# pymlex/recommendation-system-pokec

Measured on AMD Instinct MI355X. Metric: FAS candidates scored/sec over 1.6M users, top-k=10; 1/2/4/8 GPU + %HBM peak, higher is better.
Workload: dtype f64; 1 GPU; cfg2: full 1.6M-user single-query interest FAS all-candidates top-10; workload_key=cfg2_all_candidates_top10_1632803users_q1_shard1of1, topk=10, parallelism=candidate-shard x1, hw_queues=4

## Files before the change

include/pokec_fas.h:

```cpp
#ifndef POKEC_FAS_H
#define POKEC_FAS_H

#include <stdint.h>

#ifdef __cplusplus
extern "C" {
#endif

#define PF_ABI_VERSION 2

#define PF_OK          0
#define PF_EINVAL     -1
#define PF_ENODEV     -2
#define PF_ENOMEM     -3
#define PF_ENOTFOUND  -4
#define PF_EUNSUPP    -5
#define PF_EINTERNAL  -6

#define PF_NUM_FIXED   7
#define PF_MAX_COLS    64
#define PF_F_PUBLIC     0
#define PF_F_GENDER     1
#define PF_F_COMPLETION 2
#define PF_F_AGE        3
// ... 190 lines not shown
                       int32_t topk, uint64_t* d_keys, void* stream);
int pf_merge_keys_async(pf_ctx* ctx, const uint64_t* d_parts, int32_t nparts,
                        int32_t nq, int32_t topk, uint64_t* d_out, void* stream);
void pf_decode_keys(const uint64_t* keys, int32_t n, int32_t* out_uid,
                    float* out_score, int32_t* count);

typedef struct pf_layout_stats {
    int64_t n_slots;
    int64_t stream_bytes;
    int64_t header_bytes;
    int64_t alg_bytes;
    int32_t packed_tokens;
    int32_t n_tiles;
    int64_t post_bytes;
    int32_t scan_kernel;
    int32_t resident_images;
    int64_t shard_cands;
    int64_t shard_entries;
} pf_layout_stats;
int pf_layout(const pf_ctx* ctx, pf_layout_stats* out);

int pf_scan_bytes(pf_ctx* ctx, const int32_t* query_uid, int32_t nq, int64_t* out_bytes);
int pf_scan_prune_stats(pf_ctx* ctx, int64_t* out, int32_t reset);

typedef struct pf_jobs_stats {
    int64_t jobs, candidates, pairs;
    int64_t pair_alg_bytes, pair_record_bytes, pair_image_bytes;
    double  pair_ms;
    int64_t pair_launches;
    int64_t pair_dispatches;
} pf_jobs_stats;
int pf_jobs_stats_reset(pf_ctx* ctx, int32_t enable);
int pf_jobs_stats_read(pf_ctx* ctx, pf_jobs_stats* out);

float pf_last_scan_ms(const pf_ctx* ctx);
int pf_profile_reset(pf_ctx* ctx);
int pf_profile_read(pf_ctx* ctx, double* total_ms, int64_t* launches);
int pf_profile_sample(pf_ctx* ctx, int32_t every);

#ifdef __cplusplus
}
#endif
#endif
```

recommendation-system-pokec_amd/csrc/pf_api.cpp:

```cpp
#include <hip/hip_runtime.h>

#include <algorithm>
#include <atomic>
#include <cmath>
#include <cstdlib>
#include <cstring>
#include <mutex>
#include <string>
#include <thread>
#include <unordered_map>
#include <unordered_set>
#include <vector>

#include "pf_batch.h"
#include "pf_ctx.h"
#include "pf_debug.h"
#include "pf_kernels.h"
#include "pf_store.h"
#include "pokec_fas.h"

using pf::DBuf;
using pf::PinBuf;
using pf::Ranked;
using pf::par_jobs;
// ... 243 lines not shown
        HIPCHK(c, hipStreamSynchronize(c->stream));
        k.hl.lap(pf::kHpGpu);
        const pf_pair_terms_head* rh = c->h_thead.as<pf_pair_terms_head>();
        const double* rt = c->h_terms.as<double>();
        par_jobs(k.g1 - k.g0, [&](size_t i) {
            const size_t g = k.g0 + i;
            for (size_t j = 0; j < slots[g].size(); ++j) {
                head[dest[g][j]] = rh[k.gf[i] + j];
                std::memcpy(terms + (size_t)dest[g][j] * W, rt + (k.gf[i] + j) * W, W * sizeof(double));
            }
        }, 256);
        k.hl.lap(pf::kHpUnpack);
        return PF_OK;
    });
}

uint32_t post_mode(bool claimed) {
    static const long pr = pf::debug_long("k5_prune", 2);
    static const bool prb = pf::debug_long("k5_prune_batch", 1) != 0;
    static const bool prs = pf::debug_long("k5_prune_stats", 0) != 0;
    const uint32_t p = pr <= 0 ? 0u : (pf::kPostPrune | (pr == 1 ? pf::kPostPruneBlockOnly : 0u) | (prs ? pf::kPostPruneStats : 0u));
    static const bool fko = pf::debug_long("k5_filter_blockout", 1) == 0;
    const uint32_t f = fko ? pf::kPostFiltKeepBlocks : 0u;
    return ((claimed || prb) ? p : 0u) | f;
}

constexpr int kBatchBlocksPerWgDefault = 32;
int batch_blocks_per_wg() {
    static const int n = (int)std::max(1L, pf::debug_long("k5_batch_blocks", kBatchBlocksPerWgDefault));
    return n;
}

uint32_t post_image_lds(const pf::QPostHead* h) {
    return pf::post_lds(pf::post_var_lds(h->n_tok, h->n_tok + h->n_club + h->n_friend));
}
uint32_t filt_lds(const pf_ctx* c) { return (c->filt.fields ? pf::kFiltLds : 0u) + (c->win.fields ? pf::kWinLds : 0u); }

struct CountScope {
    pf_ctx* c;
    int n;
    bool on;
    CountScope(pf_ctx* ctx, int nq) : c(ctx), n(nq), on((ctx->win.fields & pf::kWinCount) != 0u && nq > 0) {}
    ~CountScope() { c->cur_totals = nullptr; }
    int begin() {
        if (!on) return PF_OK;
        HIPCHK(c, c->d_totals.ensure((size_t)n * sizeof(uint32_t)));
        HIPCHK(c, hipMemsetAsync(c->d_totals.p, 0, (size_t)n * sizeof(uint32_t), c->stream));
// ... 1262 lines not shown
}

int pf_merge_keys_async(pf_ctx* c, const uint64_t* d_parts, int32_t nparts, int32_t nq, int32_t topk, uint64_t* d_out,
                        void* stream) {
    if (!c || nparts < 1 || nq < 0 || topk <= 0 || topk > pf::kMaxTopK) return PF_EINVAL;
    (void)hipSetDevice(c->device);
    hipStream_t s = (hipStream_t)stream;
    HIPCHK(c, pf::launch_merge(d_parts, nparts, (int64_t)nq * topk, topk, nq, topk, d_out, s));
    return PF_OK;
}

int pf_jobs_stats_reset(pf_ctx* c, int32_t enable) { return c ? pf::jobs_stats_reset(c, enable) : PF_EINVAL; }
int pf_jobs_stats_read(pf_ctx* c, pf_jobs_stats* o) { return (c && o) ? pf::jobs_stats_read(c, o) : PF_EINVAL; }

int pf_scan_prune_stats(pf_ctx* c, int64_t* out, int32_t reset) {
    if (!c || !out) return PF_EINVAL;
    (void)hipSetDevice(c->device);
    unsigned long long v[5];
    HIPCHK(c, pf::k5_prune_stats_read(v, reset != 0));
    for (int i = 0; i < 5; ++i) out[i] = (int64_t)v[i];
    return PF_OK;
}

int pf_scan_bytes(pf_ctx* c, const int32_t* q, int32_t nq, int64_t* out) {
    if (!c || nq < 0 || (nq && (!q || !out))) return PF_EINVAL;
    (void)hipSetDevice(c->device);
    int64_t k1 = 0;
    for (int32_t t = c->tile_begin; t < c->tile_end; ++t) k1 += (int64_t)c->hs.tile_steps[t] * pf::kTileSlots * 16;
    k1 += (int64_t)(c->tile_end - c->tile_begin) * pf::kTileSlots * 48;
    if (!c->use_post()) {
        for (int i = 0; i < nq; ++i) out[i] = c->hc.idx_of(q[i]) < 0 ? 0 : k1;
        return PF_OK;
    }
    std::vector<std::vector<uint8_t>> imgs((size_t)nq);
    std::vector<int8_t> kind((size_t)nq, 0);
    par_jobs((size_t)nq, [&](size_t i) {
        const int32_t x = c->hc.idx_of(q[i]);
        if (x < 0) return;
        std::vector<int32_t> ex;
        auto it = c->hc.adj.find(q[i]);
        if (it != c->hc.adj.end()) ex = it->second;
        ex.push_back(q[i]);
        pf::build_query_post(c->hc, c->hp, x, ex, imgs[i]);
        const pf::QPostHead* h = reinterpret_cast<const pf::QPostHead*>(imgs[i].data() + sizeof(pf::QConst));
        kind[i] = post_image_lds(h) <= kK5LdsCap ? 1 : 2;
    }, 1);
// ... 106 lines not shown
```

recommendation-system-pokec_amd/csrc/pf_kernels.h:

```cpp
#pragma once
#include <hip/hip_runtime.h>

#include "pf_filter.h"
#include "pf_select.h"
#include "pf_types.h"
#include "pf_window.h"

namespace pf {

constexpr int kPairThreads = 512;
struct PairBlock {
    int32_t qimg, begin, count, out;
};

struct PairGen {
    int32_t nf, nch, cap, cand, fl, stride, out, first;
};

struct ScanLaunch {
    const DevStore& st;
    const uint8_t* pool;
    const QImageRef* refs_dev;
    uint32_t lds;
    bool gtab;
    int nq, tile_begin, tile_end, k, blocks;
    uint64_t *parts, *out;
    ScanSync* sync;
    const int32_t* out_rows;
    hipStream_t s;
    const CandFilter& filt;
    const FieldSel& sel;
    const ScanWindow& win;
    uint32_t* totals;
};
hipError_t launch_scan(const ScanLaunch& L);
int scan_blocks_per_cu(bool packed, bool gtab, uint32_t lds);
uint32_t post_var_lds(int n_tok, int n_lists);
uint32_t post_lds(uint32_t var_lds);
constexpr uint32_t kPostPrune = 1u << 16, kPostPruneStats = 1u << 17, kPostPruneBlockOnly = 1u << 18;
constexpr uint32_t kPostFiltKeepBlocks = 1u << 19;
constexpr uint32_t kFiltLds = (uint32_t)sizeof(CandFilter);
static_assert(kFiltLds % 16 == 0, "the window's words follow the filter's");
constexpr uint32_t kWinLds = 32;
static_assert(sizeof(ScanWindow) <= kWinLds, "the window's LDS");
struct PostLaunch {
    const PostStore& ps;
    const uint8_t* pool;
    const uint32_t* img_off;
    uint32_t var_lds;
    int nq, blk_begin, blk_end, k, blocks;
    uint64_t *parts, *out;
    ScanSync* sync;
    const int32_t* out_rows;
    bool claimed;
    uint32_t mode;
    hipEvent_t e0, e1;
    hipStream_t s;
    const uint8_t* qconst;
    const CandFilter& filt;
    const FieldSel& sel;
    const ScanWindow& win;
    uint32_t* totals;
};
hipError_t launch_post(const PostLaunch& L);
int post_blocks_per_cu(uint32_t var_lds, bool claimed, bool filtered, bool selected, bool windowed);
hipError_t launch_filter_count(const PostStore& ps, const DevStore& st, int32_t i0, int32_t i1, const CandFilter& filt,
                               unsigned long long* count, hipStream_t s);
hipError_t k5_prune_stats_read(unsigned long long* out, bool reset);
hipError_t launch_merge(const uint64_t* in, int nparts, int64_t part_stride, int64_t query_stride, int nq, int k,
                        uint64_t* out, hipStream_t s);
struct PairsLaunch {
    const DevStore& st;
    const uint8_t* pool;
    const QImageRef* refs_dev;
    uint32_t max_lds;
    bool gtab;
    const PairBlock* blocks;
    int nblocks;
    const int32_t *order, *slots;
    float* out;
    hipStream_t s;
    const FieldSel& sel;
};
hipError_t launch_pairs(const PairsLaunch& L);
constexpr int kTermsThreads = 256;
constexpr int kTermsPairs = 32;
struct TermsLaunch {
    const DevStore& st;
    const uint8_t* pool;
    const QImageRef* refs_dev;
    uint32_t lds;
// ... 13 lines not shown
```

recommendation-system-pokec_amd/csrc/pf_kernels.hip:

```cpp
#include <hip/hip_ext.h>
#include <hip/hip_runtime.h>

#include <cstdint>
#include <algorithm>
#include <unordered_map>
#include <vector>
#include <cstdio>
#include <cstdlib>

#include "pf_device.h"
#include "pf_filter.h"
#include "pf_kernels.h"
#include "pf_plan.h"
#include "pf_prune.h"
#include "pf_select.h"

namespace pf {

static_assert(sizeof(QConst) % 16 == 0, "QConst must keep the LDS carve 16-B aligned");
static_assert(sizeof(QVal) == 16, "QVal is one 16-B load");

#ifdef PF_K5_TIMERS
__device__ unsigned long long g_k5t[16];
__device__ unsigned long long g_k1t[12];
#endif

constexpr int kPruneStats = 5;
static_assert(kPruneBins <= (int)(sizeof(ScanSync::hist) / sizeof(unsigned int)), "the histogram holds every bin");
__device__ unsigned long long g_k5_prune[kPruneStats];

#ifdef PF_K5_BLOCKLOG
constexpr unsigned kBlogCap = 16384;
__device__ unsigned long long g_blog_t[2 * kBlogCap];
__device__ unsigned int g_blog_meta[kBlogCap];
__device__ unsigned int g_blog_n;
#endif

__device__ __forceinline__ void wave_sync() {
    __builtin_amdgcn_fence(__ATOMIC_RELEASE, "wavefront");
    __builtin_amdgcn_wave_barrier();
    __builtin_amdgcn_fence(__ATOMIC_ACQUIRE, "wavefront");
}

struct Walk {
    uint32_t cnt;
    uint32_t nh;
    uint32_t pend;
};

template <bool PACKED>
struct HitT;
template <>
// ... 790 lines not shown
    double wq, idf;
};

constexpr uint32_t kLdsMask = 0;
constexpr uint32_t kLdsSlot = kLdsMask + 8 * kBlockCands;
constexpr uint32_t kLdsHit = kLdsSlot + 8 * kRoundCap;
constexpr uint32_t kLdsHbase = kLdsHit + 2 * kRoundCap;
constexpr uint32_t kLdsCnt = kLdsSlot;
constexpr uint32_t kLdsExb = kLdsCnt + 4 * kBlockCands;
static_assert(4 * kBlockCands + 4 * (kBlockCands / 32) <= 8 * kRoundCap, "set counters alias the slots");
constexpr uint32_t kLdsItem = kLdsHbase + 2 * kBlockCands;
constexpr uint32_t kLdsMisc = (kLdsItem + 2 * kRoundCap + 15) & ~15u;
constexpr uint32_t kLdsCols = kLdsMisc + 64;
constexpr uint32_t kLdsFtab = kLdsCols + 16 * kPostMaxCols;
constexpr uint32_t kLdsSeg = kLdsFtab + 8 * (kNumFixed + kPostMaxCols + 1);
constexpr uint32_t kLdsCidx = kLdsSeg + 4 * kRoundToks;
constexpr uint32_t kMapWords = kRoundCap / 64;
constexpr uint32_t kLdsMapB = (kLdsCidx + 7) & ~7u;
constexpr uint32_t kLdsMapN = kLdsMapB + 2 * 8 * kMapWords;
constexpr uint32_t kLdsMapC = kLdsMapN + 2 * 8 * kRoundToks;
constexpr uint32_t kLdsLmk = (kLdsMapC + 2 * kMapWords + 7) & ~7u;
constexpr uint32_t kLdsCpre = kLdsLmk + 8 * kPostMaxCols;
constexpr uint32_t kLdsNeed = kLdsCpre + 8 * (kPostMaxCols + 1);
constexpr uint32_t kPostFixedLds = (kLdsNeed + 8 * (kNumFixed + kPostMaxCols + 1) + 15) & ~15u;
static_assert(kBlockCands == 2 * kPostThreads, "two candidates per thread");
static_assert(kRoundCap < 65536 && kBlockCands <= kRoundCap, "u16 slots; a one-token round fits");
static_assert(kPostWaves * kMaxTopK * 8 + 16 + 4 * kMaxTopK <= 8 * kRoundCap, "post_tail scratch in the slots");

constexpr uint32_t kHitFirst = 1u << 14;
constexpr uint32_t kHitCand = 1u << 15;
constexpr uint32_t kSegSplit = 1u << 24;
constexpr uint8_t kColDead = 0xFFu;

#ifdef PF_K5_CHECK
__device__ __forceinline__ uint32_t k5_chk(uint32_t i, uint32_t n, int what) {
    if (i >= n) {
        printf("K5 CHECK %d: index %u >= %u (block %d thread %d)\n", what, i, n, (int)blockIdx.x, (int)threadIdx.x);
        return 0u;
    }
    return i;
}
#define K5CHK(i, n, w) k5_chk((i), (n), (w))
#else
#define K5CHK(i, n, w) (i)
#endif


// ... 176 lines not shown
    uint16_t* hit = reinterpret_cast<uint16_t*>(base + kLdsHit);
    uint16_t* hbase = reinterpret_cast<uint16_t*>(base + kLdsHbase);
    uint16_t* item = reinterpret_cast<uint16_t*>(base + kLdsItem);
    uint32_t* cnt = reinterpret_cast<uint32_t*>(base + kLdsCnt);
    uint32_t* exb = reinterpret_cast<uint32_t*>(base + kLdsExb);
    uint32_t* misc = reinterpret_cast<uint32_t*>(base + kLdsMisc);
    QCol* scol = reinterpret_cast<QCol*>(base + kLdsCols);
    double* ftab = reinterpret_cast<double*>(base + kLdsFtab);
    uint32_t* seg = reinterpret_cast<uint32_t*>(base + kLdsSeg);
    const int nsets = H.n_club + H.n_friend;
    const int nl = H.n_tok + nsets;
    PTok* pt = reinterpret_cast<PTok*>(base + kPostFixedLds);
    uint2* rng = reinterpret_cast<uint2*>(pt + H.n_tok);
    uint2* rtab = rng + nl;
    uint32_t* gpre = reinterpret_cast<uint32_t*>(rtab + H.n_tok + 1);
    uint32_t* spre = gpre + H.n_tok + 1;
    uint8_t* colof = reinterpret_cast<uint8_t*>(spre + nsets + 1);
    uint64_t* mapb = reinterpret_cast<uint64_t*>(base + kLdsMapB);
    uint2* mapn = reinterpret_cast<uint2*>(base + kLdsMapN);
    uint8_t* mapc = reinterpret_cast<uint8_t*>(base + kLdsMapC);
    uint64_t* lmk = reinterpret_cast<uint64_t*>(base + kLdsLmk);
    uint64_t* cpre = reinterpret_cast<uint64_t*>(base + kLdsCpre);
    double* need = reinterpret_cast<double*>(base + kLdsNeed);
    const bool prune = (mode & kPostPrune) != 0u;
    const bool prune_rnd = prune && !(mode & kPostPruneBlockOnly);
    const bool pstats = (mode & kPostPruneStats) != 0u;
    const bool drop = FILT || prune;
    CandFilter* fl = reinterpret_cast<CandFilter*>(
        smem + (((uint32_t)(reinterpret_cast<char*>(colof) + H.n_tok - smem) + 15u) & ~15u));
    if constexpr (FILT) {
        if (tid == 0) *fl = F;
    }
    const ScanWindow* wl = reinterpret_cast<const ScanWindow*>(reinterpret_cast<char*>(fl) + (FILT ? kFiltLds : 0u));
    if constexpr (WIN) {
        if (tid == 0) *const_cast<ScanWindow*>(wl) = W;
    }
    if (tid < 16) misc[tid] = 0u;
    stage(smem, qcp, sizeof(QConst));
    if constexpr (!SEL) {
        for (int j = tid; j < H.n_act; j += kPostThreads) {
            const QCol c = cols[j];
            scol[j] = c;
            for (int x = c.j0; x < c.j1; ++x) colof[x] = (uint8_t)j;
        }
        if (tid == 0) {
            uint64_t m = 0;
            for (int j = 0; j < H.n_act; ++j) { cpre[j] = m; m |= 1ull << cols[j].t; }
            cpre[H.n_act] = m;
        }
// ... 41 lines not shown
    const uint32_t B = (uint32_t)ps.bsize;
    const uint32_t cend = min((uint32_t)blk_end * B, (uint32_t)ps.n);
    const bool short_excl = H.n_excl <= kPostThreads;
    const uint32_t ex0 = short_excl && H.n_excl > 0 ? excl[min(tid, H.n_excl - 1)] : ~0u;
    const int pb = (nbx & 7) == 0 ? (bx & 7) * (nbx >> 3) + (bx >> 3) : bx;
    const int xng = min(8, nbx), xg = bx % xng;
    const int x_lo = blk_begin + (int)((int64_t)(blk_end - blk_begin) * xg / xng);
    const int x_hi = blk_begin + (int)((int64_t)(blk_end - blk_begin) * (xg + 1) / xng);
    const int x_nwg = (nbx - xg + xng - 1) / xng;
    unsigned int* xctr = &sync[qy].xcd_next[xg * 16];
    const int blk_last = XD ? x_hi : blk_end;
    for (int blk = XD ? x_lo + bx / xng : blk_begin + pb; blk < blk_last;) {
        unsigned int xclaim = 0;
        auto next_block = [&](bool now) __attribute__((always_inline)) {
            if constexpr (XD) {
                if (tid == 0) misc[0] = (uint32_t)(x_lo + x_nwg) + (now ? atomicAdd(xctr, 1u) : xclaim);
                __syncthreads();
                blk = (int)misc[0];
            } else {
                __syncthreads();
                blk += nbx;
            }
        };
        const uint32_t c0 = (uint32_t)blk * B;
        const uint32_t c1 = min(c0 + B, cend) - 1;
#ifdef PF_K5_BLOCKLOG
        const unsigned long long blog_t0 = __builtin_amdgcn_s_memrealtime();
#endif
        uint4 ha[kCandsPerThread], hb[kCandsPerThread];
#pragma unroll
        for (int kk = 0; kk < kCandsPerThread; ++kk) {
            const uint32_t c = min(c0 + kk * kPostThreads + tid, c1);
            ha[kk] = ps.hdr[2 * (size_t)c];
            hb[kk] = ps.hdr[2 * (size_t)c + 1];
        }
        uint32_t thb = 0u;
        if (prune) thb = __hip_atomic_load(&sync[qy].theta, __ATOMIC_RELAXED, __HIP_MEMORY_SCOPE_AGENT);
        if constexpr (WIN) {
            if (prune) thb = max(thb, wl->theta0);
        }
#pragma unroll 1
        for (int j = tid; j < nl; j += kPostThreads)
            rng[j] = list_range(ps, j < H.n_tok ? toks[j].l : sets[j - H.n_tok], c0, c1);
#pragma unroll
        for (int kk = 0; kk < kCandsPerThread; ++kk) {
            const uint32_t c = c0 + kk * kPostThreads + tid;
// ... 24 lines not shown
                    misc[12] += thb == 0u ? 1u : 0u;
                }
                next_block(true);
                continue;
            }
#pragma unroll
            for (int kk = 0; kk < kCandsPerThread; ++kk) {
                const uint64_t bal = __ballot((fskip >> kk) & 1u);
                const uint32_t w = (uint32_t)(bal >> (lane & 32));
                if ((lane & 31) == 0 && w != 0u) atomicOr(&exb[(kk * kPostThreads + tid) >> 5], w);
            }
        } else {
            __syncthreads();
        }
        K5T(1);
        if (prune && tid >= kPostThreads - 64) {
            thb = (uint32_t)__builtin_amdgcn_readfirstlane((int)thb);
            const uint32_t rec = misc[5];
            if (rec != 0u) {
                thb = prune_derive(sync + qy, thb | (uint32_t)k, rec);
                wave_sync();
                if (lane == 0) misc[5] = 0u;
            }
            const int u = tid - (kPostThreads - 64);
            if (u == 0) misc[4] = thb;
            if (u >= 0 && u <= kNumFixed + kPostMaxCols) need[u] = prune_need(thb, u, kNumFixed + q.n_cols);
        }
        if (tid < 64) {
            ColPlan cpl = col_tokens(scol, H.n_act, lane);
            wave_prefix<SEL>(gpre, rng, H.n_tok, lane, pt);
            wave_sync();
            col_ends(cpl, gpre, H.n_act, lane);
            {
                int ci0 = 0, j0 = 0, nr = 0;
                while (ci0 < H.n_act) {
                    if constexpr (SEL) j0 = max(j0, __builtin_amdgcn_readlane(cpl.j0, ci0));
                    const Round Rr = plan_round(cpl, gpre, H.n_act, lane, ci0, j0);
                    if (lane == 0)
                        rtab[nr] = make_uint2((uint32_t)Rr.ja | (uint32_t)Rr.jb << 16, (uint32_t)Rr.ca | (uint32_t)Rr.ce << 16);
                    if (nr == 0) build_map(mapb, mapc, mapn, gpre, rng, Rr.ja, Rr.jb, lane);
                    ++nr;
                }
                if (lane == 0) misc[3] = (uint32_t)nr;
            }
        }
        if (short_excl) {
            const uint32_t p = ex0 - c0;
            if (tid < H.n_excl && p < B) atomicOr(&exb[p >> 5], 1u << (p & 31));
        } else {
            uint32_t lo = 0, hi = (uint32_t)H.n_excl;
            while (lo < hi) {
                const uint32_t mid = (lo + hi) >> 1;
                if (excl[mid] < c0) lo = mid + 1; else hi = mid;
            }
            hi = (uint32_t)H.n_excl;
// ... 50 lines not shown
        }
        if (drop) {
#pragma unroll
            for (int kk = 0; kk < kCandsPerThread; ++kk) {
                const bool sk = (skip >> kk) & 1u;
                const bool d = prune && !sk && prune_dead(sum[kk], (double)__popcll(pend[kk]), need[(used >> (8 * kk)) & 0xFFu]);
                if (sk || d) {
                    skip |= 1u << kk;
                    pend[kk] = 0ull;
                }
                if (pstats) {
                    const int p = kk * kPostThreads + tid;
                    const uint64_t bs = __ballot((uint32_t)p < B && c0 + p <= c1), bd = __ballot(d);
                    if (lane == 0) {
                        atomicAdd(&misc[8], (uint32_t)__popcll(bs));
                        atomicAdd(&misc[9], (uint32_t)__popcll(bd));
                    }
                }
            }
            if (pstats && tid == 0) {
                misc[11] += 1u;
                misc[12] += misc[4] == 0u ? 1u : 0u;
            }
        }
        K5T(3);
        double cdot[kCandsPerThread], cnrm[kCandsPerThread];
        uint32_t chit = 0;
#pragma unroll
        for (int kk = 0; kk < kCandsPerThread; ++kk) { cdot[kk] = 0.0; cnrm[kk] = 0.0; }
        int nrounds = (int)misc[3];
        if (XD && nrounds == 0 && tid == 0) xclaim = atomicAdd(xctr, 1u);
        for (int rnd = 0; rnd < nrounds; ++rnd) {
            if (XD && rnd == nrounds - 1 && tid == 0) xclaim = atomicAdd(xctr, 1u);
            const uint2 rr = rtab[rnd];
            Round R;
            R.ja = (int)(rr.x & 0xFFFFu);
            R.jb = (int)(rr.x >> 16);
            R.ca = (int)(rr.y & 0xFFFFu);
            R.ce = (int)(rr.y >> 16);
            const int mbuf = rnd & 1;
            const int ja = R.ja, jb = R.jb;
            const uint32_t g0 = gpre[ja], F = gpre[jb] - g0;
            if (F > 0) {
                if (tid < jb - ja) {
                    const int j = ja + tid;
                    const QCol c = scol[SEL ? min((int)colof[j], kPostMaxCols - 1) : (int)colof[j]];
                    const int lo = max(c.j0, ja) - ja, hi = min(c.j1, jb) - ja;
                    seg[tid] = (uint32_t)lo | (uint32_t)hi << 8 | (uint32_t)c.t << 16 |
                               ((c.j0 < ja || c.j1 > jb) ? kSegSplit : 0u);
                }
                if (tid < R.ce - R.ca) {
                    const QCol c = scol[R.ca + tid];
                    lmk[c.t] = low_bits((uint32_t)(min((int)c.j1, jb) - ja));
                }
                if (tid == 0) misc[1] = 0u;
                constexpr int U = kRoundCap / kPostThreads;
                uint32_t kp[U];
                double kn[U];
                {
                    uint32_t xs[U];
                    int js[U];
                    uint32_t ft = (uint32_t)tid;
                    asm volatile("" : "+v"(ft));
#pragma unroll
                    for (int u = 0; u < U; ++u) {
                        const uint32_t f = ft + (uint32_t)(kPostThreads * u);
                        js[u] = -1;
                        xs[u] = 0u;
                        if (f < F) {
                            const uint32_t w = f >> 6;
                            const uint32_t kk = (uint32_t)mapc[mbuf * kMapWords + w] +
                                                (uint32_t)__popcll(mapb[mbuf * kMapWords + w] & low_bits((f & 63u) + 1u)) - 1u;
                            const uint2 L = mapn[mbuf * kRoundToks + kk];
                            js[u] = ja + (int)L.y;
                            xs[u] = L.x + f;
                        }
                    }
                    uint32_t ent[U];
#pragma unroll
                    for (int u = 0; u < U; ++u) {
                        ent[u] = ps.post[K5CHK(xs[u], ps.n_tok_entries, 4)];
                        kn[u] = ps.pnorm[K5CHK(xs[u], ps.n_tok_entries, 5)];
                    }
#pragma unroll
                    for (int u = 0; u < U; ++u) {
                        const uint32_t p = (ent[u] >> 8) - c0;
                        kp[u] = ~0u;
                        if (js[u] >= 0 && p < B) {
                            const uint32_t jr = (uint32_t)(js[u] - ja);
                            kp[u] = p | jr << 10 | (ent[u] & 0xFFu) << 16;
                            atomicOr(reinterpret_cast<unsigned long long*>(&mask[p]), 1ull << jr);
                        }
                    }
                }
                for (uint32_t f = (uint32_t)(tid + kRoundCap); f < F; f += kPostThreads) {
                    const int j = round_list(gpre, ja, jb, g0 + f);
                    const uint32_t p = (ps.post[K5CHK(rng[j].x + (g0 + f - gpre[j]), ps.n_tok_entries, 6)] >> 8) - c0;
                    if (p < B) atomicOr(reinterpret_cast<unsigned long long*>(&mask[p]), 1ull << (j - ja));
                }
                K5T(4);
                __syncthreads();
                K5T(5);
                if (tid < 64 && rnd + 1 < nrounds) {
                    const uint2 r1 = rtab[rnd + 1];
                    const int nb = mbuf ^ 1;
                    build_map(mapb + nb * kMapWords, mapc + nb * kMapWords, mapn + nb * kRoundToks, gpre, rng,
                              (int)(r1.x & 0xFFFFu), (int)(r1.x >> 16), lane);
                }
                uint32_t nk[kCandsPerThread], tot = 0;
#pragma unroll
                for (int kk = 0; kk < kCandsPerThread; ++kk) {
                    uint64_t m = mask[kk * kPostThreads + tid];
                    if (drop && ((skip >> kk) & 1u) && m != 0ull) {
                        mask[kk * kPostThreads + tid] = 0ull;
                        m = 0ull;
                    }
                    nk[kk] = (uint32_t)__popcll(m);
                    tot += nk[kk];
                }
                uint32_t incl = tot;
                incl = wave_incl_scan(incl);
                const uint32_t wn = wave_last(incl);
                uint32_t wb = 0;
                if (lane == 0) wb = atomicAdd(&misc[1], wn);
                wb = (uint32_t)__shfl((int)wb, 0);
                {
                    uint32_t h0 = wb + incl - tot;
#pragma unroll
                    for (int kk = 0; kk < kCandsPerThread; ++kk) {
                        hbase[kk * kPostThreads + tid] = (uint16_t)h0;
                        h0 += nk[kk];
                    }
                }
                K5T(6);
                __syncthreads();
                K5T(1);
#pragma unroll
                for (int u = 0; u < U; ++u) {
                    if (kp[u] == ~0u) continue;
                    const uint32_t p = kp[u] & 1023u, jr = (kp[u] >> 10) & 63u, tf = kp[u] >> 16;
                    if (drop && !((mask[p] >> jr) & 1ull)) continue;
                    const uint64_t below = mask[p] & low_bits(jr);
                    const uint32_t r = K5CHK(hbase[p] + (uint32_t)__popcll(below), (uint32_t)kRoundCap, 8);
                    const uint32_t sg = seg[jr], lo = sg & 0xFFu;
                    const bool first = (below >> lo) == 0ull;
                    hit[r] = (uint16_t)(tf | jr << 8 | (first ? kHitFirst : 0u) | (below == 0ull ? kHitCand : 0u));
                    slot[r] = first ? kn[u] : tok_product(pt, ja + (int)jr, tf);
                    item[r] = (first && !(sg & kSegSplit)) ? (uint16_t)hit_run(mask[p], lo, (sg >> 8) & 0xFFu) : (uint16_t)0;
                }
                for (uint32_t f = (uint32_t)(tid + kRoundCap); f < F; f += kPostThreads) {
                    const int j = round_list(gpre, ja, jb, g0 + f);
                    const uint32_t x = K5CHK(rng[j].x + (g0 + f - gpre[j]), ps.n_tok_entries, 7);
                    const uint32_t e = ps.post[x];
                    const uint32_t p = (e >> 8) - c0;
                    if (p >= B) continue;
                    const uint32_t jr = (uint32_t)(j - ja);
                    if (drop && !((mask[p] >> jr) & 1ull)) continue;
                    const uint64_t below = mask[p] & low_bits(jr);
                    const uint32_t r = K5CHK(hbase[p] + (uint32_t)__popcll(below), (uint32_t)kRoundCap, 9);
                    const uint32_t sg = seg[jr];
                    const bool first = (below >> (sg & 0xFFu)) == 0ull;
                    hit[r] = (uint16_t)((e & 0xFFu) | jr << 8 | (first ? kHitFirst : 0u) | (below == 0ull ? kHitCand : 0u));
                    slot[r] = first ? ps.pnorm[x] : tok_product(pt, ja + (int)jr, e & 0xFFu);
                    item[r] = (first && !(sg & kSegSplit)) ? (uint16_t)hit_run(mask[p], sg & 0xFFu, (sg >> 8) & 0xFFu) : (uint16_t)0;
                }
                K5T(7);
                __syncthreads();
                K5T(8);
                {
                uint16_t* wit = item + wb;
                uint32_t ni = 0;
                for (uint32_t r0 = wb; r0 < wb + wn; r0 += 64) {
// ... 68 lines not shown
                    if (t != t_on) {
                        const bool hh = (chit >> kk) & 1u;
                        sum[kk] += (hh && cdot[kk] != 0.0) ? text_term(q, t, cdot[kk], cnrm[kk]) : q.sig0_col[t];
                        cdot[kk] = 0.0;
                        chit &= ~(1u << kk);
                    }
                }
                if (F > 0) mask[p] = 0ull;
            }
            if (prune_rnd && rnd + 1 < nrounds) {
                const uint64_t togo = ~(cpre[R.ce] & ~(t_on >= 0 ? 1ull << t_on : 0ull));
#pragma unroll
                for (int kk = 0; kk < kCandsPerThread; ++kk) {
                    const bool d = !((skip >> kk) & 1u) &&
                                   prune_dead(sum[kk], (double)__popcll(pend[kk] & togo), need[(used >> (8 * kk)) & 0xFFu]);
                    if (d) {
                        skip |= 1u << kk;
                        pend[kk] = 0ull;
                    }
                    if (pstats) {
                        const uint64_t bal = __ballot(d);
                        if (lane == 0) atomicAdd(&misc[10], (uint32_t)__popcll(bal));
                    }
                }
            }
            K5T(10);
            if (F == 0 && rnd + 1 < nrounds) {
                if (tid < 64) {
                    const uint2 r1 = rtab[rnd + 1];
                    const int nb = mbuf ^ 1;
                    build_map(mapb + nb * kMapWords, mapc + nb * kMapWords, mapn + nb * kRoundToks, gpre, rng,
                              (int)(r1.x & 0xFFFFu), (int)(r1.x >> 16), lane);
                }
                __syncthreads();
            }
            if (F > 0) __syncthreads();
        }
        K5T(11);
        uint64_t keys[kCandsPerThread];
#pragma unroll
        for (int kk = 0; kk < kCandsPerThread; ++kk) {
            uint64_t key = ~0ull;
            if (!((skip >> kk) & 1u)) {
                const int uk = (int)((used >> (8 * kk)) & 0xFFu);
                const float f = fas_score(sum[kk], uk, ftab[uk]);
                key = score_key(f, (int32_t)(c0 + kk * kPostThreads + tid));
                if constexpr (WIN) {
                    if (!window_pass(key, *wl)) key = ~0ull;
// ... 3 lines not shown
        }
        if constexpr (WIN) {
            if (wl->fields & kWinCount) {
                const uint32_t nin = (uint32_t)__popcll(__ballot(keys[0] != ~0ull)) + (uint32_t)__popcll(__ballot(keys[1] != ~0ull));
                if (lane == 0 && nin != 0u) atomicAdd(&misc[6], nin);
            }
        }
        static_assert(kCandsPerThread == 2, "2-key sort");
        if (keys[1] < keys[0]) { const uint64_t x = keys[0]; keys[0] = keys[1]; keys[1] = x; }
#pragma unroll
        for (int kk = 0; kk < kCandsPerThread; ++kk) topk_push(best, keys[kk], k, lane);
        if (prune && !(WIN && (wl->fields & kWinCount))) prune_fold(&misc[5], best, k, c0, c1, misc[4], lane);
        K5T(12);
#ifdef PF_K5_BLOCKLOG
        if (tid == 0) {
            const unsigned i = atomicAdd(&g_blog_n, 1u);
            if (i < kBlogCap) {
                g_blog_t[2 * i] = blog_t0;
                g_blog_t[2 * i + 1] = __builtin_amdgcn_s_memrealtime();
                g_blog_meta[i] = (unsigned)bx | (unsigned)blk << 16;
            }
        }
#endif
        next_block(false);
    }
    if (prune && tid == kPostThreads - 64) {
        const uint32_t rec = misc[5];
        if (rec != 0u) {
            const uint32_t old = __hip_atomic_fetch_add(&sync[qy].hist[prune_bin(rec)], 1u, __ATOMIC_RELAXED, __HIP_MEMORY_SCOPE_AGENT);
            asm volatile("" ::"v"(old));
        }
    }
#ifdef PF_K5_TIMERS
    tacc[13] = clock64() - tstart;
    if (lane == 0) {
        for (int i = 0; i < 14; ++i) atomicAdd(&g_k5t[i], (unsigned long long)tacc[i]);
        atomicAdd(&g_k5t[15], 1ull);
    }
#endif
    if (pstats) {
        __syncthreads();
        if (tid < kPruneStats) atomicAdd(&g_k5_prune[tid], (unsigned long long)misc[8 + tid]);
    }
    if (lane < k && best != ~0ull) {
        const uint32_t idx = (uint32_t)best ^ 0x80000000u;
        best = (best & 0xFFFFFFFF00000000ull) | (ps.hdr[2 * (size_t)idx + 1].w ^ 0x80000000u);
    }
    uint64_t* sc = reinterpret_cast<uint64_t*>(slot);

    if constexpr (WIN) {
        const bool counted = (wl->fields & kWinCount) != 0u;
        post_tail(best, k, sc, sync, parts, out, out_rows, qy, bx, nbx, counted, tid == 0 ? misc[6] : 0u, totals);
    } else {
        post_tail(best, k, sc, sync, parts, out, out_rows, qy, bx, nbx);
    }
}

constexpr int kMergeThreads = 1024;
__global__ __launch_bounds__(kMergeThreads) void topk_merge_kernel(const uint64_t* __restrict__ in, int32_t nparts,
                                                                   int64_t part_stride, int64_t query_stride, int32_t k,
                                                                   uint64_t* __restrict__ out,
                                                                   const int32_t* __restrict__ out_rows) {
    __shared__ uint64_t sc[16 * 64];
    const int q = blockIdx.x, lane = threadIdx.x & 63, wave = threadIdx.x >> 6;
    const int64_t total = (int64_t)nparts * k;
// ... 238 lines not shown
                                     "total"};
        if (++calls % 10 == 0) {
            fprintf(stderr, "k5t per wave (clock64):");
            for (int i = 0; i < 14; ++i) fprintf(stderr, " %s=%.0f", nm[i], (double)t[i] / (double)t[15]);
            fprintf(stderr, "\n");
        }
        const unsigned long long z[16] = {0};
        hipMemcpyToSymbol(HIP_SYMBOL(g_k5t), z, sizeof(z));
    }
#endif
    return hipGetLastError();
}

hipError_t k5_prune_stats_read(unsigned long long* out, bool reset) {
    hipError_t e = hipDeviceSynchronize();
    if (e == hipSuccess) e = hipMemcpyFromSymbol(out, HIP_SYMBOL(g_k5_prune), kPruneStats * sizeof(unsigned long long));
    if (e == hipSuccess && reset) {
        const unsigned long long z[kPruneStats] = {0};
        e = hipMemcpyToSymbol(HIP_SYMBOL(g_k5_prune), z, sizeof(z));
    }
    return e;
}

int post_blocks_per_cu(uint32_t var_lds, bool claimed, bool filtered, bool selected, bool windowed) {
    static thread_local std::unordered_map<uint32_t, int> memos[16];
    auto& memo = memos[8 * (int)windowed + 4 * (int)selected + 2 * (int)filtered + (int)claimed];
    auto it = memo.find(var_lds);
    if (it != memo.end()) return it->second;
    int nb = 0;
    const size_t lds = post_lds(var_lds) + (filtered ? kFiltLds : 0u) + (windowed ? kWinLds : 0u);
    const hipError_t e = hipOccupancyMaxActiveBlocksPerMultiprocessor(&nb, post_kernel(claimed, filtered, selected, windowed), kPostThreads, lds);
    nb =(e == hipSuccess && nb > 0) ? nb : 1;
    if (memo.size() > 4096) memo.clear();
    memo.emplace(var_lds, nb);
    return nb;
}

hipError_t launch_merge(const uint64_t* in, int nparts, int64_t part_stride, int64_t query_stride, int nq, int k,
                        uint64_t* out, hipStream_t s) {
    if (nq <= 0) return hipSuccess;
    hipLaunchKernelGGL(topk_merge_kernel, dim3(nq), dim3(kMergeThreads), 0, s, in, nparts, part_stride, query_stride,
                       k, out, (const int32_t*)nullptr);
    return hipGetLastError();
}

hipError_t launch_pairs(const PairsLaunch& L) {
// ... 29 lines not shown
```

recommendation-system-pokec_amd/pokec_fas.py:

```python
import contextlib
import ctypes
import os

import numpy as np

HERE = os.path.dirname(os.path.abspath(__file__))
LIB_PATH = os.environ.get("PF_LIB_PATH") or os.path.join(HERE, "libpokec_fas.so")

PF_OK, PF_EINVAL, PF_ENODEV, PF_ENOMEM, PF_ENOTFOUND, PF_EUNSUPP = 0, -1, -2, -3, -4, -5
PF_MODE_FOF, PF_MODE_ALL = 0, 1
PF_FOF_GRAPH, PF_FOF_COLLAB = 0, 1
PF_SCAN_AUTO, PF_SCAN_STREAM, PF_SCAN_POSTINGS = 0, 1, 2
MAX_TOPK_DEVICE = 64
PF_FILT_GENDER, PF_FILT_PUBLIC, PF_FILT_AGE, PF_FILT_COMPLETION, PF_FILT_REGION = 1, 2, 4, 8, 16
PF_FILT_KEEP_MISSING = 1
PF_F_PUBLIC, PF_F_GENDER, PF_F_COMPLETION, PF_F_AGE, PF_F_REGION, PF_F_CLUBS, PF_F_FRIENDS = range(7)
PF_SEL_FIXED_ALL = 0x7F
PF_WIN_MIN, PF_WIN_AFTER, PF_WIN_COUNT = 1, 2, 4
FIXED_FIELD_NAMES = ("public", "gender", "completion", "age", "region", "clubs", "friends")

EXPORTS = ["pf_abi_version", "pf_open", "pf_close", "pf_last_error", "pf_num_users", "pf_idf", "pf_fas_pairs",
           "pf_recommend_interest", "pf_recommend_collab", "pf_recommend_clubs", "pf_fof_candidates", "pf_set_adj",
           "pf_set_shard", "pf_scan_keys_async", "pf_merge_keys_async", "pf_decode_keys", "pf_layout",
           "pf_last_scan_ms", "pf_profile_reset", "pf_profile_read", "pf_profile_sample", "pf_set_scan_kernel",
           "pf_scan_bytes", "pf_scan_prune_stats", "pf_jobs_stats_reset", "pf_jobs_stats_read", "pf_recommend_interest_async",
           "pf_recommend_collab_async", "pf_recommend_clubs_async", "pf_wait", "pf_completed_ticket",
           "pf_set_scan_filter", "pf_scan_filter_count", "pf_set_scan_select", "pf_fas_pairs_select",
           "pf_num_cols", "pf_fas_pairs_terms", "pf_recommend_interest_all_terms",
           "pf_recommend_interest_profile", "pf_fas_profile_pairs", "pf_fas_profile_pairs_terms",
           "pf_recommend_interest_profile_terms",
           "pf_recommend_group", "pf_group_scores", "pf_group_plan_of", "pf_group_image_lds",
           "pf_set_scan_window", "pf_scan_window_totals"]
IO_EXPORTS = ["pf_dataset_load", "pf_dataset_load_cached", "pf_dataset_free", "pf_dataset_desc", "pf_dataset_info_get", "pf_dataset_column",
              "pf_dataset_profile_order", "pf_dataset_adj_order", "pf_dataset_profile_json", "pf_dataset_club_name",
              "pf_compute_normalizers", "pf_holdout_friends", "pf_recommendation_tests",
              "pf_eval_holdout_friends", "pf_eval_recommendation_tests", "pf_holdout_friends_digest",
              "pf_recommendation_tests_digest", "pf_eval_holdout_friends_digest",
              "pf_eval_recommendation_tests_digest", "pf_eval_recommendation_tests_async"]
PF_LOAD_REFERENCE_CAP = 100000


class PfLayoutStats(ctypes.Structure):
    _fields_ = [("n_slots", ctypes.c_int64), ("stream_bytes", ctypes.c_int64), ("header_bytes", ctypes.c_int64),
                ("alg_bytes", ctypes.c_int64), ("packed_tokens", ctypes.c_int32), ("n_tiles", ctypes.c_int32),
                ("post_bytes", ctypes.c_int64), ("scan_kernel", ctypes.c_int32), ("resident_images", ctypes.c_int32),
                ("shard_cands", ctypes.c_int64), ("shard_entries", ctypes.c_int64)]


class CandFilter(ctypes.Structure):
    _fields_ = [("fields", ctypes.c_uint32), ("flags", ctypes.c_uint32), ("gender", ctypes.c_int32),
                ("public_flag", ctypes.c_int32), ("age_min", ctypes.c_int32), ("age_max", ctypes.c_int32),
                ("completion_min", ctypes.c_int32), ("completion_max", ctypes.c_int32),
                ("region", ctypes.c_int32 * 3), ("pad", ctypes.c_int32)]

    @classmethod
# ... 290 lines not shown
        L.pf_recommend_interest_all_terms.argtypes = [V, V, I32, I32, V, V, V, V, V]
        L.pf_recommend_interest_profile.argtypes = [V, V, I32, I32, V, V, V]
        L.pf_fas_profile_pairs.argtypes = [V, V, V, I64, ctypes.POINTER(FieldSelect), V]
        L.pf_fas_profile_pairs_terms.argtypes = [V, V, V, I64, ctypes.POINTER(FieldSelect), V, V]
        L.pf_recommend_interest_profile_terms.argtypes = [V, V, I32, I32, V, V, V, V, V]
        L.pf_scan_keys_async.argtypes = [V, V, I32, I32, V, V]
        L.pf_recommend_group.argtypes = [V, ctypes.POINTER(GroupQuery), I32, I32, V, V, V]
        L.pf_group_scores.argtypes = [V, ctypes.POINTER(GroupQuery), V, I64, ctypes.POINTER(FieldSelect), V]
        L.pf_group_plan_of.argtypes = [V, ctypes.POINTER(GroupQuery), ctypes.POINTER(GroupPlan)]
        L.pf_group_image_lds.argtypes = [V, ctypes.POINTER(GroupQuery), V, I32]
        L.pf_set_scan_window.argtypes = [V, ctypes.POINTER(ScanWindow)]
        L.pf_scan_window_totals.argtypes = [V, V, I32, ctypes.POINTER(I32)]
        L.pf_merge_keys_async.argtypes = [V, V, I32, I32, I32, V, V]
        L.pf_decode_keys.argtypes = [V, I32, V, V, V]
        L.pf_decode_keys.restype = None
        L.pf_layout.argtypes = [V, ctypes.POINTER(PfLayoutStats)]
        L.pf_last_scan_ms.argtypes = [V]
        L.pf_last_scan_ms.restype = ctypes.c_float
        L.pf_profile_reset.argtypes = [V]
        L.pf_profile_sample.argtypes = [V, I32]
        L.pf_profile_read.argtypes = [V, ctypes.POINTER(ctypes.c_double), ctypes.POINTER(I64)]
        L.pf_scan_bytes.argtypes = [V, V, I32, V]
        L.pf_scan_prune_stats.argtypes = [V, V, I32]
        L.pf_jobs_stats_reset.argtypes = [V, I32]
        L.pf_jobs_stats_read.argtypes = [V, ctypes.POINTER(PfJobsStats)]
        L.pf_dataset_load.argtypes = [ctypes.c_char_p, I64, ctypes.POINTER(V)]
        L.pf_dataset_load_cached.argtypes = [ctypes.c_char_p, I64, ctypes.c_char_p, ctypes.POINTER(I32), ctypes.POINTER(V)]
        L.pf_dataset_free.argtypes = [V]
        L.pf_dataset_free.restype = None
        L.pf_dataset_desc.argtypes = [V]
        L.pf_dataset_desc.restype = V
        L.pf_dataset_info_get.argtypes = [V, ctypes.POINTER(PfDatasetInfo)]
        L.pf_dataset_column.argtypes = [V, I32]
        L.pf_dataset_column.restype = ctypes.c_char_p
        L.pf_dataset_profile_order.argtypes = [V, V, I32, ctypes.POINTER(I32)]
        L.pf_dataset_adj_order.argtypes = [V, V, I32, ctypes.POINTER(I32)]
        L.pf_dataset_profile_json.argtypes = [V, I32, V, I64, ctypes.POINTER(I64)]
        L.pf_dataset_club_name.argtypes = [V, I32]
        L.pf_dataset_club_name.restype = ctypes.c_char_p
        L.pf_compute_normalizers.argtypes = [V, I32, I32, ctypes.c_char_p, V, V]
        L.pf_holdout_friends.argtypes = [V, V, I32, V, I32, ctypes.POINTER(I32)]
        L.pf_recommendation_tests.argtypes = [V, V, I32, I32, V]
        L.pf_eval_holdout_friends.argtypes = [V, V, I32, I32, I32, I32, V, I32, ctypes.POINTER(I32)]
        L.pf_eval_recommendation_tests.argtypes = [V, V, I32, I32, I32, I32, I32, V, V, I32, ctypes.POINTER(I32)]
        L.pf_holdout_friends_digest.argtypes = [V, V, I32, V, I32, ctypes.POINTER(I32)]
        L.pf_recommendation_tests_digest.argtypes = [V, V, I32, I32, V, I32, ctypes.POINTER(I32)]
# ... 360 lines not shown

    def profile_sample(self, every):
        self._check(self._L.pf_profile_sample(self.h, int(every)), "pf_profile_sample")

    def profile_read(self):
        ms, n = ctypes.c_double(), ctypes.c_int64()
        self._check(self._L.pf_profile_read(self.h, ctypes.byref(ms), ctypes.byref(n)), "pf_profile_read")
        return ms.value, n.value

    def jobs_stats_reset(self, time_pairs=True, count=True):
        self._check(self._L.pf_jobs_stats_reset(self.h, (1 if time_pairs else 0) | (2 if count else 0)),
                    "pf_jobs_stats_reset")

    def jobs_stats(self):
        s = PfJobsStats()
        self._check(self._L.pf_jobs_stats_read(self.h, ctypes.byref(s)), "pf_jobs_stats_read")
        return {k: getattr(s, k) for k, _ in PfJobsStats._fields_}

    def k5_prune_stats(self, reset=False):
        out = np.zeros(5, np.int64)
        self._check(self._L.pf_scan_prune_stats(self.h, out.ctypes.data, 1 if reset else 0), "pf_scan_prune_stats")
        return dict(zip(("seen", "dead_block_start", "dead_round_end", "blocks", "cold_blocks"), (int(x) for x in out)))

    def scan_bytes(self, uids):
        q = np.ascontiguousarray(np.atleast_1d(uids), np.int32)
        out = np.zeros(len(q), np.int64)
        self._check(self._L.pf_scan_bytes(self.h, q.ctypes.data, len(q), out.ctypes.data), "pf_scan_bytes")
        return out


def decode_keys(keys):
    keys = np.ascontiguousarray(keys, np.uint64)
    ou = np.zeros(len(keys), np.int32)
    os_ = np.zeros(len(keys), np.float32)
    n = ctypes.c_int32()
    lib().pf_decode_keys(keys.ctypes.data, len(keys), ou.ctypes.data, os_.ctypes.data, ctypes.byref(n))
    return ou[:n.value], os_[:n.value]


class Dataset:

    def __init__(self, root, max_lines=PF_LOAD_REFERENCE_CAP, cache=None):
        L = lib()
        self._L = L
        self.h = ctypes.c_void_p()
        fc = ctypes.c_int32(0)
# ... 185 lines not shown
```

Before: 17.13 billion candidates/s.

## Exit posting rounds early once every block candidate is pruned, defer norm loads

Adds a per-block LDS bitmap of dead candidates, written by ballot after pruning. The round loop breaks early once no live candidate remains, so later posting rounds are not walked. Posting-norm loads are moved after the mask check so only first-hit entries fetch pnorm. It also adds optional walk-statistics counters and an API to read them. The cost is extra LDS, ballots and syncs per round, plus a changed next_block hint when rounds are skipped.

```diff
diff --git a/include/pokec_fas.h b/include/pokec_fas.h
--- a/include/pokec_fas.h
+++ b/include/pokec_fas.h
@@ -236,6 +236,7 @@
 
 int pf_scan_bytes(pf_ctx* ctx, const int32_t* query_uid, int32_t nq, int64_t* out_bytes);
 int pf_scan_prune_stats(pf_ctx* ctx, int64_t* out, int32_t reset);
+int pf_scan_walk_stats(pf_ctx* ctx, int64_t* out, int32_t reset);
 
 typedef struct pf_jobs_stats {
     int64_t jobs, candidates, pairs;
diff --git a/recommendation-system-pokec_amd/csrc/pf_api.cpp b/recommendation-system-pokec_amd/csrc/pf_api.cpp
--- a/recommendation-system-pokec_amd/csrc/pf_api.cpp
+++ b/recommendation-system-pokec_amd/csrc/pf_api.cpp
@@ -289,7 +289,7 @@
     const uint32_t p = pr <= 0 ? 0u : (pf::kPostPrune | (pr == 1 ? pf::kPostPruneBlockOnly : 0u) | (prs ? pf::kPostPruneStats : 0u));
     static const bool fko = pf::debug_long("k5_filter_blockout", 1) == 0;
     const uint32_t f = fko ? pf::kPostFiltKeepBlocks : 0u;
-    return ((claimed || prb) ? p : 0u) | f;
+    return ((claimed || prb) ? p : 0u) | f | (prs ? pf::kPostWalkStats : 0u);
 }
 
 constexpr int kBatchBlocksPerWgDefault = 32;
@@ -1598,6 +1598,15 @@
     return PF_OK;
 }
 
+int pf_scan_walk_stats(pf_ctx* c, int64_t* out, int32_t reset) {
+    if (!c || !out) return PF_EINVAL;
+    (void)hipSetDevice(c->device);
+    unsigned long long v[3];
+    HIPCHK(c, pf::k5_walk_stats_read(v, reset != 0));
+    for (int i = 0; i < 3; ++i) out[i] = (int64_t)v[i];
+    return PF_OK;
+}
+
 int pf_scan_bytes(pf_ctx* c, const int32_t* q, int32_t nq, int64_t* out) {
     if (!c || nq < 0 || (nq && (!q || !out))) return PF_EINVAL;
     (void)hipSetDevice(c->device);
diff --git a/recommendation-system-pokec_amd/csrc/pf_kernels.h b/recommendation-system-pokec_amd/csrc/pf_kernels.h
--- a/recommendation-system-pokec_amd/csrc/pf_kernels.h
+++ b/recommendation-system-pokec_amd/csrc/pf_kernels.h
@@ -39,6 +39,7 @@
 uint32_t post_lds(uint32_t var_lds);
 constexpr uint32_t kPostPrune = 1u << 16, kPostPruneStats = 1u << 17, kPostPruneBlockOnly = 1u << 18;
 constexpr uint32_t kPostFiltKeepBlocks = 1u << 19;
+constexpr uint32_t kPostWalkStats = 1u << 20;
 constexpr uint32_t kFiltLds = (uint32_t)sizeof(CandFilter);
 static_assert(kFiltLds % 16 == 0, "the window's words follow the filter's");
 constexpr uint32_t kWinLds = 32;
@@ -67,6 +68,7 @@
 hipError_t launch_filter_count(const PostStore& ps, const DevStore& st, int32_t i0, int32_t i1, const CandFilter& filt,
                                unsigned long long* count, hipStream_t s);
 hipError_t k5_prune_stats_read(unsigned long long* out, bool reset);
+hipError_t k5_walk_stats_read(unsigned long long* out, bool reset);
 hipError_t launch_merge(const uint64_t* in, int nparts, int64_t part_stride, int64_t query_stride, int nq, int k,
                         uint64_t* out, hipStream_t s);
 struct PairsLaunch {
diff --git a/recommendation-system-pokec_amd/csrc/pf_kernels.hip b/recommendation-system-pokec_amd/csrc/pf_kernels.hip
--- a/recommendation-system-pokec_amd/csrc/pf_kernels.hip
+++ b/recommendation-system-pokec_amd/csrc/pf_kernels.hip
@@ -26,8 +26,9 @@
 #endif
 
 constexpr int kPruneStats = 5;
+constexpr int kWalkStats = 3;
 static_assert(kPruneBins <= (int)(sizeof(ScanSync::hist) / sizeof(unsigned int)), "the histogram holds every bin");
-__device__ unsigned long long g_k5_prune[kPruneStats];
+__device__ unsigned long long g_k5_prune[kPruneStats + kWalkStats];
 
 #ifdef PF_K5_BLOCKLOG
 constexpr unsigned kBlogCap = 16384;
@@ -864,7 +865,9 @@
 constexpr uint32_t kLdsLmk = (kLdsMapC + 2 * kMapWords + 7) & ~7u;
 constexpr uint32_t kLdsCpre = kLdsLmk + 8 * kPostMaxCols;
 constexpr uint32_t kLdsNeed = kLdsCpre + 8 * (kPostMaxCols + 1);
-constexpr uint32_t kPostFixedLds = (kLdsNeed + 8 * (kNumFixed + kPostMaxCols + 1) + 15) & ~15u;
+constexpr uint32_t kLdsDead = kLdsNeed + 8 * (kNumFixed + kPostMaxCols + 1);
+constexpr uint32_t kPostFixedLds = (kLdsDead + 8 * (kBlockCands / 64) + 15) & ~15u;
+static_assert(kBlockCands / 64 <= 64, "one lane per word of the dead bitmap");
 static_assert(kBlockCands == 2 * kPostThreads, "two candidates per thread");
 static_assert(kRoundCap < 65536 && kBlockCands <= kRoundCap, "u16 slots; a one-token round fits");
 static_assert(kPostWaves * kMaxTopK * 8 + 16 + 4 * kMaxTopK <= 8 * kRoundCap, "post_tail scratch in the slots");
@@ -1087,9 +1090,11 @@
     uint64_t* lmk = reinterpret_cast<uint64_t*>(base + kLdsLmk);
     uint64_t* cpre = reinterpret_cast<uint64_t*>(base + kLdsCpre);
     double* need = reinterpret_cast<double*>(base + kLdsNeed);
+    uint64_t* dead = reinterpret_cast<uint64_t*>(base + kLdsDead);
     const bool prune = (mode & kPostPrune) != 0u;
     const bool prune_rnd = prune && !(mode & kPostPruneBlockOnly);
     const bool pstats = (mode & kPostPruneStats) != 0u;
+    const bool wstats = (mode & kPostWalkStats) != 0u;
     const bool drop = FILT || prune;
     CandFilter* fl = reinterpret_cast<CandFilter*>(
         smem + (((uint32_t)(reinterpret_cast<char*>(colof) + H.n_tok - smem) + 15u) & ~15u));
@@ -1177,6 +1182,11 @@
                 blk += nbx;
             }
         };
+        auto dead_put = [&](int kk, uint64_t bal) __attribute__((always_inline)) {
+            uint32_t w = (uint32_t)tid >> 6;
+            asm volatile("" : "+v"(w));
+            if (lane == 0) dead[kk * (kPostThreads / 64) + (int)w] = bal;
+        };
         const uint32_t c0 = (uint32_t)blk * B;
         const uint32_t c1 = min(c0 + B, cend) - 1;
 #ifdef PF_K5_BLOCKLOG
@@ -1247,15 +1257,18 @@
                 wave_sync();
                 if (lane == 0) misc[5] = 0u;
             }
-            const int u = tid - (kPostThreads - 64);
+            int u = tid - (kPostThreads - 64);
+            asm volatile("" : "+v"(u));
             if (u == 0) misc[4] = thb;
             if (u >= 0 && u <= kNumFixed + kPostMaxCols) need[u] = prune_need(thb, u, kNumFixed + q.n_cols);
         }
         if (tid < 64) {
-            ColPlan cpl = col_tokens(scol, H.n_act, lane);
-            wave_prefix<SEL>(gpre, rng, H.n_tok, lane, pt);
+            int pl = lane;
+            asm volatile("" : "+v"(pl));
+            ColPlan cpl = col_tokens(scol, H.n_act, pl);
+            wave_prefix<SEL>(gpre, rng, H.n_tok, pl, pt);
             wave_sync();
-            col_ends(cpl, gpre, H.n_act, lane);
+            col_ends(cpl, gpre, H.n_act, pl);
             {
                 int ci0 = 0, j0 = 0, nr = 0;
                 while (ci0 < H.n_act) {
@@ -1352,15 +1365,31 @@
                 misc[11] += 1u;
                 misc[12] += misc[4] == 0u ? 1u : 0u;
             }
-        }
+#pragma unroll
+            for (int kk = 0; kk < kCandsPerThread; ++kk) {
+                dead_put(kk, __ballot((skip >> kk) & 1u));
+            }
+        }
+        auto nobody_left = [&]() __attribute__((always_inline)) {
+            uint32_t w = (uint32_t)lane & (uint32_t)(kBlockCands / 64 - 1);
+            asm volatile("" : "+v"(w));
+            return __ballot(dead[w] != ~0ull) == 0ull;
+        };
+        static_assert((kBlockCands / 64 & (kBlockCands / 64 - 1)) == 0, "the bitmap's words by lane");
         K5T(3);
         double cdot[kCandsPerThread], cnrm[kCandsPerThread];
         uint32_t chit = 0;
 #pragma unroll
         for (int kk = 0; kk < kCandsPerThread; ++kk) { cdot[kk] = 0.0; cnrm[kk] = 0.0; }
         int nrounds = (int)misc[3];
+        bool ahead = nrounds == 0;
         if (XD && nrounds == 0 && tid == 0) xclaim = atomicAdd(xctr, 1u);
         for (int rnd = 0; rnd < nrounds; ++rnd) {
+            if (drop && rnd > 0 && nobody_left()) {
+                if (wstats && tid == 0) misc[15] += (uint32_t)(nrounds - rnd);
+                break;
+            }
+            if (rnd == nrounds - 1) ahead = true;
             if (XD && rnd == nrounds - 1 && tid == 0) xclaim = atomicAdd(xctr, 1u);
             const uint2 rr = rtab[rnd];
             Round R;
@@ -1386,9 +1415,8 @@
                 if (tid == 0) misc[1] = 0u;
                 constexpr int U = kRoundCap / kPostThreads;
                 uint32_t kp[U];
-                double kn[U];
+                uint32_t xs[U];
                 {
-                    uint32_t xs[U];
                     int js[U];
                     uint32_t ft = (uint32_t)tid;
                     asm volatile("" : "+v"(ft));
@@ -1410,7 +1438,6 @@
 #pragma unroll
                     for (int u = 0; u < U; ++u) {
                         ent[u] = ps.post[K5CHK(xs[u], ps.n_tok_entries, 4)];
-                        kn[u] = ps.pnorm[K5CHK(xs[u], ps.n_tok_entries, 5)];
                     }
 #pragma unroll
                     for (int u = 0; u < U; ++u) {
@@ -1431,6 +1458,10 @@
                 K5T(4);
                 __syncthreads();
                 K5T(5);
+                if (drop && rnd == 0 && nobody_left()) {
+                    if (wstats && tid == 0) misc[15] += (uint32_t)nrounds;
+                    break;
+                }
                 if (tid < 64 && rnd + 1 < nrounds) {
                     const uint2 r1 = rtab[rnd + 1];
                     const int nb = mbuf ^ 1;
@@ -1465,19 +1496,37 @@
                 K5T(6);
                 __syncthreads();
                 K5T(1);
+                double kn[U];
 #pragma unroll
                 for (int u = 0; u < U; ++u) {
-                    if (kp[u] == ~0u) continue;
-                    const uint32_t p = kp[u] & 1023u, jr = (kp[u] >> 10) & 63u, tf = kp[u] >> 16;
-                    if (drop && !((mask[p] >> jr) & 1ull)) continue;
-                    const uint64_t below = mask[p] & low_bits(jr);
-                    const uint32_t r = K5CHK(hbase[p] + (uint32_t)__popcll(below), (uint32_t)kRoundCap, 8);
-                    const uint32_t sg = seg[jr], lo = sg & 0xFFu;
-                    const bool first = (below >> lo) == 0ull;
-                    hit[r] = (uint16_t)(tf | jr << 8 | (first ? kHitFirst : 0u) | (below == 0ull ? kHitCand : 0u));
-                    slot[r] = first ? kn[u] : tok_product(pt, ja + (int)jr, tf);
-                    item[r] = (first && !(sg & kSegSplit)) ? (uint16_t)hit_run(mask[p], lo, (sg >> 8) & 0xFFu) : (uint16_t)0;
-                }
+                    uint32_t x = 0u, rs = ~0u;
+                    if (kp[u] != ~0u) {
+                        const uint32_t p = kp[u] & 1023u, jr = (kp[u] >> 10) & 63u, tf = kp[u] >> 16;
+                        if (!drop || ((mask[p] >> jr) & 1ull)) {
+                            const uint64_t below = mask[p] & low_bits(jr);
+                            const uint32_t r = K5CHK(hbase[p] + (uint32_t)__popcll(below), (uint32_t)kRoundCap, 8);
+                            const uint32_t sg = seg[jr], lo = sg & 0xFFu;
+                            const bool first = (below >> lo) == 0ull;
+                            hit[r] = (uint16_t)(tf | jr << 8 | (first ? kHitFirst : 0u) | (below == 0ull ? kHitCand : 0u));
+                            item[r] = (first && !(sg & kSegSplit)) ? (uint16_t)hit_run(mask[p], lo, (sg >> 8) & 0xFFu) : (uint16_t)0;
+                            if (first) {
+                                x = K5CHK(xs[u], ps.n_tok_entries, 5);
+                                rs = r;
+                            } else {
+                                slot[r] = tok_product(pt, ja + (int)jr, tf);
+                            }
+                        }
+                    }
+                    kn[u] = ps.pnorm[x];
+                    xs[u] = rs;
+                    if (wstats) {
+                        const uint64_t bal = __ballot(rs != ~0u);
+                        if (lane == 0 && bal != 0ull) atomicAdd(&misc[13], (uint32_t)__popcll(bal));
+                    }
+                }
+#pragma unroll
+                for (int u = 0; u < U; ++u)
+                    if (xs[u] != ~0u) slot[xs[u]] = kn[u];
                 for (uint32_t f = (uint32_t)(tid + kRoundCap); f < F; f += kPostThreads) {
                     const int j = round_list(gpre, ja, jb, g0 + f);
                     const uint32_t x = K5CHK(rng[j].x + (g0 + f - gpre[j]), ps.n_tok_entries, 7);
@@ -1592,8 +1641,10 @@
                         const uint64_t bal = __ballot(d);
                         if (lane == 0) atomicAdd(&misc[10], (uint32_t)__popcll(bal));
                     }
-                }
-            }
+                    dead_put(kk, __ballot((skip >> kk) & 1u));
+                }
+            }
+            if (wstats && tid == 0) misc[14] += 1u;
             K5T(10);
             if (F == 0 && rnd + 1 < nrounds) {
                 if (tid < 64) {
@@ -1643,7 +1694,7 @@
             }
         }
 #endif
-        next_block(false);
+        next_block(!ahead);
     }
     if (prune && tid == kPostThreads - 64) {
         const uint32_t rec = misc[5];
@@ -1659,9 +1710,9 @@
         atomicAdd(&g_k5t[15], 1ull);
     }
 #endif
-    if (pstats) {
+    if (pstats || wstats) {
         __syncthreads();
-        if (tid < kPruneStats) atomicAdd(&g_k5_prune[tid], (unsigned long long)misc[8 + tid]);
+        if (tid < kPruneStats + kWalkStats) atomicAdd(&g_k5_prune[tid], (unsigned long long)misc[8 + tid]);
     }
     if (lane < k && best != ~0ull) {
         const uint32_t idx = (uint32_t)best ^ 0x80000000u;
@@ -1946,6 +1997,17 @@
     return e;
 }
 
+hipError_t k5_walk_stats_read(unsigned long long* out, bool reset) {
+    constexpr size_t off = kPruneStats * sizeof(unsigned long long);
+    hipError_t e = hipDeviceSynchronize();
+    if (e == hipSuccess) e = hipMemcpyFromSymbol(out, HIP_SYMBOL(g_k5_prune), kWalkStats * sizeof(unsigned long long), off);
+    if (e == hipSuccess && reset) {
+        const unsigned long long z[kWalkStats] = {0};
+        e = hipMemcpyToSymbol(HIP_SYMBOL(g_k5_prune), z, sizeof(z), off);
+    }
+    return e;
+}
+
 int post_blocks_per_cu(uint32_t var_lds, bool claimed, bool filtered, bool selected, bool windowed) {
     static thread_local std::unordered_map<uint32_t, int> memos[16];
     auto& memo = memos[8 * (int)windowed + 4 * (int)selected + 2 * (int)filtered + (int)claimed];
diff --git a/recommendation-system-pokec_amd/pokec_fas.py b/recommendation-system-pokec_amd/pokec_fas.py
--- a/recommendation-system-pokec_amd/pokec_fas.py
+++ b/recommendation-system-pokec_amd/pokec_fas.py
@@ -30,7 +30,7 @@
            "pf_recommend_interest_profile", "pf_fas_profile_pairs", "pf_fas_profile_pairs_terms",
            "pf_recommend_interest_profile_terms",
            "pf_recommend_group", "pf_group_scores", "pf_group_plan_of", "pf_group_image_lds",
-           "pf_set_scan_window", "pf_scan_window_totals"]
+           "pf_set_scan_window", "pf_scan_window_totals", "pf_scan_walk_stats"]
 IO_EXPORTS = ["pf_dataset_load", "pf_dataset_load_cached", "pf_dataset_free", "pf_dataset_desc", "pf_dataset_info_get", "pf_dataset_column",
               "pf_dataset_profile_order", "pf_dataset_adj_order", "pf_dataset_profile_json", "pf_dataset_club_name",
               "pf_compute_normalizers", "pf_holdout_friends", "pf_recommendation_tests",
@@ -367,6 +367,7 @@
         L.pf_profile_read.argtypes = [V, ctypes.POINTER(ctypes.c_double), ctypes.POINTER(I64)]
         L.pf_scan_bytes.argtypes = [V, V, I32, V]
         L.pf_scan_prune_stats.argtypes = [V, V, I32]
+        L.pf_scan_walk_stats.argtypes = [V, V, I32]
         L.pf_jobs_stats_reset.argtypes = [V, I32]
         L.pf_jobs_stats_read.argtypes = [V, ctypes.POINTER(PfJobsStats)]
         L.pf_dataset_load.argtypes = [ctypes.c_char_p, I64, ctypes.POINTER(V)]
@@ -773,6 +774,11 @@
         self._check(self._L.pf_scan_prune_stats(self.h, out.ctypes.data, 1 if reset else 0), "pf_scan_prune_stats")
         return dict(zip(("seen", "dead_block_start", "dead_round_end", "blocks", "cold_blocks"), (int(x) for x in out)))
 
+    def k5_walk_stats(self, reset=False):
+        out = np.zeros(3, np.int64)
+        self._check(self._L.pf_scan_walk_stats(self.h, out.ctypes.data, 1 if reset else 0), "pf_scan_walk_stats")
+        return dict(zip(("norms_loaded", "rounds_run", "rounds_left"), (int(x) for x in out)))
+
     def scan_bytes(self, uids):
         q = np.ascontiguousarray(np.atleast_1d(uids), np.int32)
         out = np.zeros(len(q), np.int64)
```

New measurement: 17.30 billion candidates/s, median of 5. 1.0% higher.
